# uingei/hevc

Hardware: AMD Instinct MI355X
Metric: encoded 1080p30 frames/sec/GPU; PSNR-Y parity vs libx265 at matched bitrate (higher is better)
Workload: dtype u8; 1 GPU; 1920x1080@30 SDR 8-bit Main, crf 19 capped by VBV maxrate 2940 kbps / bufsize 3528 kbit (the reference's libx265 operating point), 300-frame synthetic 'motion' clip per GPU, keyint 90 (4 closed GOPs of equal length), IPPP, full-search +-15, one clip per GPU, input resident in HBM

## Files before the change

hevc_amd/csrc/kernels/inter.h:

```cpp
#pragma once
#include "common.h"
#include "residual.h"

namespace mihevc {

template <typename T> struct InterArgs {
    Plane<const T> src[3];
    Plane<const T> ref[3];
    Plane<T> rec[3];
    int w, h, ctus_w;
    CostParams prm;
    const int16_t *centers;
    int32_t *me;
    mihevc_cu_rec *cu;
    int16_t *coef[3];
    unsigned long long *est;
    int sparse_coef;
    IpInfo *ip;
    Plane<const T> ref1[3];
    const int16_t *centers1;
    int32_t *me1;
};
template <typename T> DEV InterArgs<T> list1_view(const InterArgs<T> &a)
{
    InterArgs<T> b = a;
    for (int i = 0; i < 3; i++) b.ref[i] = a.ref1[i];
    b.centers = a.centers1; b.me = a.me1;
    return b;
}

DEVCONST int8_t kOff[9][2] = {{0, 0}, {-1, -1}, {0, -1}, {1, -1}, {-1, 0}, {1, 0}, {-1, 1}, {0, 1}, {1, 1}};
DEVCONST int8_t kRingSlot[8] = {4, 5, 2, 7, 1, 3, 6, 8};

template <typename T> struct PreArgs {
    Plane<const T> src, ref;
    uint8_t *lsrc, *lref;
    int w, h, bit_depth;
    int16_t *centers;
    unsigned *cost;
};
template <typename T> DEV void lowres_sample(const PreArgs<T> &a, int i)
{
    const int lw = a.w >> 2, n = lw * (a.h >> 2), sh = a.bit_depth - 8;
    if (i >= 2 * n) return;
    const Plane<const T> &p = i < n ? a.src : a.ref;
    const int k = i < n ? i : i - n, x = k % lw, y = k / lw;
    int s = 8 << sh;
#pragma unroll
    for (int j = 0; j < 4; j++) {
        const T *row = p.p + (ptrdiff_t)(4 * y + j) * p.stride + 4 * x;
        if (sizeof(T) == 1) {
            s = (int)sad_packed_u8(load_u32(row), 0u, (uint32_t)s);
        } else
            s += (int)row[0] + (int)row[1] + (int)row[2] + (int)row[3];
    }
    s >>= 4 + sh;
    (i < n ? a.lsrc : a.lref)[k] = (uint8_t)(s < 255 ? s : 255);
}
constexpr int PRE_SPAN = 2 * PRE_RANGE + 1;
constexpr int PRE_WIN_W = 40;
constexpr int PRE_WIN_STRIDE = 96;
struct PreShared {
    uint8_t blk[64];
    uint8_t win[(8 + 2 * PRE_RANGE) * PRE_WIN_STRIDE + 16];
    unsigned long long best;
    unsigned sad0;
};
template <typename T, class Ex> DEV void pre_search_program(Ex &ex, PreShared &s, const PreArgs<T> &a, int ctu)
{
    constexpr int R = PRE_RANGE, span = PRE_SPAN;
    const int lw = a.w >> 2, lh = a.h >> 2, wc = (lw + 7) >> 3, cx = ctu % wc, cy = ctu / wc;
    const int bw = lw - 8 * cx < 8 ? lw - 8 * cx : 8, bh = lh - 8 * cy < 8 ? lh - 8 * cy : 8;
    ex.phase([&](int tid) {
        if (tid < 64) { const int x = tid & 7, y = tid >> 3; s.blk[tid] = (x < bw && y < bh) ? a.lsrc[(8 * cy + y) * lw + 8 * cx + x] : (uint8_t)0; }
        if (8 * cx - R >= 0 && 8 * cx - R + PRE_WIN_W <= lw && 8 * cy - R >= 0 && 8 * cy + 8 + R <= lh) {
            constexpr int DPR = PRE_WIN_W / 4, ND = (8 + 2 * PRE_RANGE) * DPR, IT = (ND + NT - 1) / NT;
            uint32_t v[IT];
#pragma unroll
            for (int k = 0; k < IT; k++) {
                const int i = tid + k * NT;
                if (i < ND) v[k] = load_u32(a.lref + (size_t)(8 * cy - R + i / DPR) * lw + 8 * cx - R + 4 * (i % DPR));
            }
#pragma unroll
            for (int k = 0; k < IT; k++) {
                const int i = tid + k * NT;
                if (i < ND) store_u32_aligned(s.win + (i / DPR) * PRE_WIN_STRIDE + 4 * (i % DPR), v[k]);
            }
        } else {
            constexpr int NW = (8 + 2 * PRE_RANGE) * PRE_WIN_W, IT = (NW + NT - 1) / NT;
            uint8_t v[IT];
#pragma unroll
            for (int k = 0; k < IT; k++) {
                const int i = tid + k * NT;
                if (i < NW) v[k] = a.lref[clip3(0, lh - 1, 8 * cy + i / PRE_WIN_W - R) * lw + clip3(0, lw - 1, 8 * cx + i % PRE_WIN_W - R)];
            }
#pragma unroll
            for (int k = 0; k < IT; k++) {
                const int i = tid + k * NT;
                if (i < NW) s.win[(i / PRE_WIN_W) * PRE_WIN_STRIDE + i % PRE_WIN_W] = v[k];
            }
        }
        if (tid == 0) s.best = ~0ull;
    });
    ex.phase([&](int tid) {
        unsigned long long best = ~0ull;
        if (bw == 8 && bh == 8) {
            if (tid < 8 * span) {
                const int q = tid & 7, dyi = tid >> 3;
                uint64_t acc = 0;
#pragma unroll
                for (int y = 0; y < 8; y++) {
                    const uint8_t *w = s.win + (y + dyi) * PRE_WIN_STRIDE + 4 * q;
                    const uint32_t r0 = load_u32_aligned(w), r1 = load_u32_aligned(w + 4), r2 = load_u32_aligned(w + 8);
                    acc = qsad_u8(((uint64_t)r1 << 32) | r0, load_u32_aligned(s.blk + 8 * y), acc);
                    acc = qsad_u8(((uint64_t)r2 << 32) | r1, load_u32_aligned(s.blk + 8 * y + 4), acc);
                }
#pragma unroll
                for (int j = 0; j < 4; j++) {
                    const int dxi = 4 * q + j;
                    if (dxi >= span) continue;
                    const unsigned sad = (unsigned)((acc >> (16 * j)) & 0xffff);
                    if (dxi == R && dyi == R) s.sad0 = sad;
                    const unsigned long long key = ((unsigned long long)(4 * sad + (unsigned)(iabs(dxi - R) + iabs(dyi - R))) << 12) | (unsigned)(dyi * span + dxi);
                    best = key < best ? key : best;
                }
            }
        } else {
            for (int p = tid; p < span * span; p += NT) {
                const int dxi = p % span, dyi = p / span;
                unsigned sad = 0;
                for (int y = 0; y < bh; y++)
                    for (int x = 0; x < bw; x++) sad += (unsigned)iabs((int)s.blk[y * 8 + x] - (int)s.win[(y + dyi) * PRE_WIN_STRIDE + x + dxi]);
                if (dxi == R && dyi == R) s.sad0 = sad;
                const unsigned long long key = ((unsigned long long)(4 * sad + (unsigned)(iabs(dxi - R) + iabs(dyi - R))) << 12) | (unsigned)p;
                best = key < best ? key : best;
            }
        }
        if (best != ~0ull) ex.atomic_min(&s.best, best);
    });
    ex.phase([&](int tid) {
        if (tid != 0) return;
        int p = (int)(s.best & 4095);
        const unsigned sad_best = (unsigned)(((s.best >> 12) - (unsigned)(iabs(p % span - R) + iabs(p / span - R))) >> 2);
        if (2 * sad_best >= s.sad0) p = R * span + R;
        a.centers[2 * ctu] = (int16_t)(4 * (p % span - R));
        a.centers[2 * ctu + 1] = (int16_t)(4 * (p / span - R));
        if (a.cost) a.cost[ctu] = sad_best;
    });
}

DEV bool mv_rows_ok(int y, int n, int my, int h, int top, int bottom)
{
    const int ly0 = y + (my >> 2) - ((my & 3) ? 3 : 0), ly1 = y + n - 1 + (my >> 2) + ((my & 3) ? 4 : 0);
    const int cy0 = (y >> 1) + (my >> 3) - ((my & 7) ? 1 : 0), cy1 = (y >> 1) + (n >> 1) - 1 + (my >> 3) + ((my & 7) ? 2 : 0);
    if (top && (ly0 < 0 || cy0 < 0)) return false;
    if (bottom && (ly1 > h - 1 || cy1 > (h >> 1) - 1)) return false;
    return true;
}
DEV int clamp_center_y(int sy, int y0, int R, int h, int top, int bottom)
{
    const int ctu_h = h - y0 < CTU ? h - y0 : CTU;
    if (bottom && sy > h - (y0 + ctu_h) - R) sy = h - (y0 + ctu_h) - R;
    if (top && sy < R - y0) sy = R - y0;
    return sy;
}

template <typename T> struct MeShared {
    uint8_t src[32 * 32];
    unsigned long long best[21];
    uint8_t valid[21];
    unsigned nodeok[2 * MAX_RANGE + 1];
};
HDI int me_spanx(int R) { return ((2 * R + 1) + 3) & ~3; }
HDI int me_win_w(int R) { return 32 + me_spanx(R); }
HDI int me_win_stride(int R)
{
    int u = (me_win_w(R) + 4 + 3) >> 2;
    while ((u & 15) != 8) u++;
    return u << 2;
}
HDI int me_win_elems(int R) { return (32 + 2 * R) * me_win_stride(R) + 16; }

DEV void quad_block_row(const uint8_t *src, const uint8_t *ref, int ws, unsigned (&out)[4][4])
{
    uint64_t acc[4] = {0, 0, 0, 0};
// ... 143 lines not shown
                o[0] = 4 * (sx + p % spanx - R); o[1] = 4 * (sy + p / spanx - R); o[2] = (int32_t)(s.best[tid] >> 16);
            } else { o[0] = 0; o[1] = 0; o[2] = -1; }
        }
    });
}

template <typename T> struct InterShared {
    ResidualShared rs;
    T src[1536];
    T pred[1536];
    int mvx[21], mvy[21];
    unsigned cost[21];
    uint8_t valid[21];
    int satd[3][1][16];
    unsigned nsum[21];
    unsigned fsum[8][21];
    unsigned long long rbest[21];
    unsigned j16[4];
    int use16[4], use32;
    uint8_t alias[3][16];
    int tile_mvx[16], tile_mvy[16];
    uint8_t tile_node[16];
    uint8_t chosen[21];
    unsigned est;
    unsigned ip_cost, ip_act, ip_tiles;
    unsigned long long ip_sse;
    unsigned tu_dc[3][16], tu_dz[3][16], tu_bits[3][16], tu_zero[3];
};
constexpr int FRAC_PAIR_SUM = 8 * NT;
constexpr int FRAC_SCRATCH = FRAC_PAIR_SUM + NT;
static_assert(FRAC_SCRATCH <= (int)(sizeof(ResidualShared::scratch) / 4), "the fractional search's exchange must fit rs.scratch");
HDI int mc_win_y(int R) { return (32 + 2 * (R + 3) + 8 + 3) & ~3; }
HDI int mc_win_y_stride(int R) { return mc_win_y(R) + 4; }
HDI int mc_win_c(int R) { return (16 + (R + 3) + 8 + 3) & ~3; }
HDI int mc_win_c_stride(int R) { return mc_win_c(R) + 4; }
template <typename T> HDI size_t mc_win_y_bytes(int R) { return ((size_t)mc_win_y(R) * mc_win_y_stride(R) + 16) * sizeof(T); }
template <typename T> HDI size_t mc_win_c_bytes(int R) { return ((size_t)mc_win_c(R) * mc_win_c_stride(R) + 16) * sizeof(T); }
HDI constexpr size_t align16(size_t v) { return (v + 15) & ~(size_t)15; }

struct BiShared {
    int mx0[21], my0[21];
    unsigned c0[21], cb[21];
    uint8_t mode[21];
    uint8_t tile_mode[16];
    int tile_mv1x[16], tile_mv1y[16];
    alignas(16) int16_t p0[1536];
};

struct InterLds { size_t y, u, v, bytes; };
template <typename T> HDI constexpr size_t inter_win_in() { return offsetof(InterShared<T>, rs) + offsetof(ResidualShared, scratch) + 4 * (size_t)FRAC_SCRATCH; }
template <typename T> HDI constexpr size_t inter_win_out() { return align16(sizeof(InterShared<T>)); }
template <typename T> HDI InterLds inter_lds(int R)
{
    const size_t n[3] = {mc_win_y_bytes<T>(R), mc_win_c_bytes<T>(R), mc_win_c_bytes<T>(R)};
    const size_t hi = offsetof(InterShared<T>, rs) + offsetof(ResidualShared, scratch) + sizeof(ResidualShared::scratch);
    size_t in = inter_win_in<T>(), out = inter_win_out<T>(), at[3];
    for (int i = 0; i < 3; i++) {
        const size_t r = align16(n[i]);
        if (in + r <= hi) { at[i] = in; in += r; } else { at[i] = out; out += r; }
    }
    return InterLds{at[0], at[1], at[2], out};
}
struct InterBLds { size_t y, u, v, bi, bytes; };
template <typename T> HDI InterBLds inter_b_lds(int R)
{
    InterBLds l;
    l.y = inter_win_out<T>();
    l.u = l.y + align16(mc_win_y_bytes<T>(R));
    l.v = l.u + align16(mc_win_c_bytes<T>(R));
    l.bi = l.v + align16(mc_win_c_bytes<T>(R));
    l.bytes = l.bi + align16(sizeof(BiShared));
    return l;
}

struct TapBytes { uint32_t lo, hi; };
struct TapPairs { uint32_t p[4]; };
DEV TapBytes tap_bytes(int f) { return TapBytes{load_u32(&g_tab.luma_tap[f][0]), load_u32(&g_tab.luma_tap[f][4])}; }
DEV TapPairs tap_pairs(int f)
{
    TapPairs t;
#pragma unroll
    for (int k = 0; k < 4; k++) t.p[k] = pack_lo16(g_tab.luma_tap[f][2 * k], g_tab.luma_tap[f][2 * k + 1]);
    return t;
}
template <typename T> DEV auto row_taps(int f)
{
    if constexpr (sizeof(T) == 1) return tap_bytes(f); else return tap_pairs(f);
}

DEV void luma_row4(const uint8_t *win, int idx, const TapBytes &t, int, int (&hv)[4])
{
    const int off = idx & 3;
    const uint8_t *p = win + (idx - off);
    uint32_t d[4], q[3];
#pragma unroll
    for (int k = 0; k < 4; k++) d[k] = load_u32_aligned(p + 4 * k);
#pragma unroll
    for (int k = 0; k < 3; k++) q[k] = align_bytes(d[k + 1], d[k], off) ^ 0x80808080u;
    hv[0] = dot4_i8(q[0], t.lo, dot4_i8(q[1], t.hi, 128 * 64));
#pragma unroll
    for (int i = 1; i < 4; i++) hv[i] = dot4_i8(align_bytes(q[1], q[0], i), t.lo, dot4_i8(align_bytes(q[2], q[1], i), t.hi, 128 * 64));
}
DEV void luma_row4(const uint16_t *win, int idx, const TapPairs &t, int shift1, int (&hv)[4])
{
    const int off = idx & 1;
    const uint16_t *p = win + (idx - off);
    uint32_t d[7], e[6], o[5];
#pragma unroll
    for (int k = 0; k < 7; k++) d[k] = load_u32_aligned(p + 2 * k);
#pragma unroll
    for (int k = 0; k < 6; k++) e[k] = align_bytes(d[k + 1], d[k], 2 * off);
#pragma unroll
    for (int k = 0; k < 5; k++) o[k] = align_bytes(e[k + 1], e[k], 2);
#pragma unroll
    for (int i = 0; i < 4; i++) {
        int v = 0;
#pragma unroll
        for (int k = 0; k < 4; k++) v = dot2_i16((i & 1) ? o[(i >> 1) + k] : e[(i >> 1) + k], t.p[k], v);
        hv[i] = v >> shift1;
    }
}

template <typename T> DEV void luma_quad14(const T *win, int i00, int ws, int fx, int fy, int bit_depth, int (&out)[4])
{
    const auto tx = row_taps<T>(fx);
    const int8_t *ty = g_tab.luma_tap[fy];
    int acc[4] = {0, 0, 0, 0};
#pragma unroll
    for (int r = 0; r < 8; r++) {
        int hv[4];
        luma_row4(win, i00 + (r - 3) * ws - 3, tx, bit_depth - 8, hv);
        const int t = ty[r];
#pragma unroll
        for (int i = 0; i < 4; i++) acc[i] += t * hv[i];
    }
#pragma unroll
    for (int i = 0; i < 4; i++) out[i] = acc[i] >> 6;
}
template <typename T> DEV int chroma_sample14(const T *p00, int ws, int fx, int fy, int bit_depth)
{
    const int8_t *tx = g_tab.chroma_tap[fx], *ty = g_tab.chroma_tap[fy];
    const int shift1 = bit_depth - 8;
    int acc = 0;
    for (int r = 0; r < 4; r++) {
        const T *row = p00 + (r - 1) * ws - 1;
        int v = tx[0] * row[0] + tx[1] * row[1] + tx[2] * row[2] + tx[3] * row[3];
        acc += ty[r] * (v >> shift1);
    }
    return acc >> 6;
}
DEV int weighted_uni(int p, int bit_depth) { const int sh = 14 - bit_depth; return clip3(0, (1 << bit_depth) - 1, (p + (1 << (sh - 1))) >> sh); }
DEV int weighted_bi(int p0, int p1, int bit_depth) { const int sh = 15 - bit_depth; return clip3(0, (1 << bit_depth) - 1, (p0 + p1 + (1 << (sh - 1))) >> sh); }

DEV void luma_col_pair(int r, const int (&hv)[4], int (&prev)[4], const TapPairs &ty, int (&acc)[8][4])
{
    if (r > 0) {
#pragma unroll
        for (int i = 0; i < 4; i++) {
            const uint32_t pr = pack_lo16(prev[i], hv[i]);
#pragma unroll
            for (int k = 0; k < 4; k++) {
                const int j = r - 1 - 2 * k;
                if (j >= 0 && j < 8) acc[j][i] = dot2_i16(pr, ty.p[k], acc[j][i]);
            }
        }
    }
#pragma unroll
    for (int i = 0; i < 4; i++) prev[i] = hv[i];
}
DEV void luma_half_diff(const uint8_t *win, int i00, int ws, int fx, int fy, int, const uint8_t *src, int src_stride, int (&m)[8][4])
{
    const TapBytes tx = tap_bytes(fx);
    if (wave_all(fy == 0)) {
#pragma unroll
        for (int j = 0; j < 8; j++) {
            int hv[4];
            luma_row4(win, i00 + j * ws - 3, tx, 0, hv);
            const uint32_t w = load_u32_aligned(src + j * src_stride);
#pragma unroll
            for (int i = 0; i < 4; i++) m[j][i] = (int)((w >> (8 * i)) & 255) - clip3(0, 255, (hv[i] + 32) >> 6);
        }
        return;
    }
    if (wave_all(fx == 0)) {
        const TapBytes ty = tap_bytes(fy);
        const int idx = i00 - 3 * ws, off = idx & 3;
        uint32_t rows[15];
#pragma unroll
        for (int r = 0; r < 15; r++) {
            const uint8_t *p = win + (idx - off) + r * ws;
            rows[r] = align_bytes(load_u32_aligned(p + 4), load_u32_aligned(p), off) ^ 0x80808080u;
        }
        uint32_t col[4][4];
#pragma unroll
        for (int g = 0; g < 4; g++) {
            const uint32_t r4[4] = {rows[4 * g], rows[4 * g + 1], rows[4 * g + 2], g < 3 ? rows[4 * g + 3] : 0u};
            transpose_bytes4(r4, col[g]);
        }
#pragma unroll
        for (int j = 0; j < 8; j++) {
            const int g = j >> 2, sh = j & 3;
            const uint32_t w = load_u32_aligned(src + j * src_stride);
#pragma unroll
            for (int i = 0; i < 4; i++) {
                const uint32_t lo = align_bytes(col[g + 1][i], col[g][i], sh), hi = align_bytes(col[g + 2][i], col[g + 1][i], sh);
                const int v = dot4_i8(lo, ty.lo, dot4_i8(hi, ty.hi, 128 * 64));
                m[j][i] = (int)((w >> (8 * i)) & 255) - clip3(0, 255, (v + 32) >> 6);
            }
        }
        return;
    }
    const TapPairs ty = tap_pairs(fy);
    int acc[8][4], prev[4];
#pragma unroll
    for (int j = 0; j < 8; j++)
#pragma unroll
        for (int i = 0; i < 4; i++) acc[j][i] = 0;
#pragma unroll
    for (int r = 0; r < 15; r++) {
        int hv[4];
        luma_row4(win, i00 + (r - 3) * ws - 3, tx, 0, hv);
        luma_col_pair(r, hv, prev, ty, acc);
    }
#pragma unroll
    for (int j = 0; j < 8; j++) {
        const uint32_t w = load_u32_aligned(src + j * src_stride);
#pragma unroll
        for (int i = 0; i < 4; i++) m[j][i] = (int)((w >> (8 * i)) & 255) - clip3(0, 255, ((acc[j][i] >> 6) + 32) >> 6);
    }
}
DEV void luma_half_diff(const uint16_t *win, int i00, int ws, int fx, int fy, int bit_depth, const uint16_t *src, int src_stride, int (&m)[8][4])
{
    const TapPairs tx = tap_pairs(fx), ty = tap_pairs(fy);
    const int shift1 = bit_depth - 8, shift3 = 14 - bit_depth, maxv = (1 << bit_depth) - 1, off3 = 1 << (shift3 - 1);
    if (wave_all(fy == 0)) {
#pragma unroll
        for (int j = 0; j < 8; j++) {
            int hv[4];
            luma_row4(win, i00 + j * ws - 3, tx, shift1, hv);
#pragma unroll
            for (int i = 0; i < 4; i++) m[j][i] = (int)src[j * src_stride + i] - clip3(0, maxv, (hv[i] + off3) >> shift3);
        }
        return;
    }
    const bool v_only = wave_all(fx == 0);
    int acc[8][4], prev[4];
#pragma unroll
    for (int j = 0; j < 8; j++)
#pragma unroll
        for (int i = 0; i < 4; i++) acc[j][i] = 0;
#pragma unroll
    for (int r = 0; r < 15; r++) {
        int hv[4];
        if (v_only) {
#pragma unroll
            for (int i = 0; i < 4; i++) hv[i] = (int)win[i00 + (r - 3) * ws + i] << (6 - shift1);
        } else luma_row4(win, i00 + (r - 3) * ws - 3, tx, shift1, hv);
        luma_col_pair(r, hv, prev, ty, acc);
    }
#pragma unroll
    for (int j = 0; j < 8; j++)
#pragma unroll
        for (int i = 0; i < 4; i++) m[j][i] = (int)src[j * src_stride + i] - clip3(0, maxv, ((acc[j][i] >> 6) + off3) >> shift3);
}
DEV void hadamard_half(int (&m)[8][4])
{
#pragma unroll
    for (int x = 0; x < 4; x++)
#pragma unroll
        for (int st = 1; st < 8; st <<= 1)
#pragma unroll
            for (int i = 0; i < 8; i++)
                if (!(i & st)) { int p = m[i][x], q = m[i + st][x]; m[i][x] = p + q; m[i + st][x] = p - q; }
#pragma unroll
    for (int y = 0; y < 8; y++) {
        const int p0 = m[y][0] + m[y][1], p1 = m[y][0] - m[y][1], p2 = m[y][2] + m[y][3], p3 = m[y][2] - m[y][3];
        m[y][0] = p0 + p2; m[y][1] = p1 + p3; m[y][2] = p0 - p2; m[y][3] = p1 - p3;
    }
}

template <typename T> DEV int luma_tile_int(const T *win, int i00, int ws, const T *src, int src_stride)
{
    int m[8][8];
#pragma unroll
    for (int j = 0; j < 8; j++) {
        int px[8];
        load_row8(win, i00 + j * ws, px);
#pragma unroll
        for (int i = 0; i < 8; i++) m[j][i] = (int)src[j * src_stride + i] - px[i];
    }
    return hadamard8_satd(m);
}

template <typename T, class Ex, bool BI = false>
DEV void inter_ctu_program(Ex &ex, InterShared<T> &s, T *win_y, T *win_u, T *win_v, const InterArgs<T> &a, int ctu, BiShared *bsh = nullptr)
{
    const int R0 = a.prm.me_range, R = R0 + 3, bd = a.prm.bit_depth, lam = a.prm.lambda_sad_q4;
    const int x0 = (ctu % a.ctus_w) * CTU, y0 = (ctu / a.ctus_w) * CTU;
    const int mct = a.prm.mc_top, mcb = a.prm.mc_bottom;
    const int sx = wave_uniform(a.centers ? a.centers[2 * ctu] : 0), sy0 = wave_uniform(a.centers ? a.centers[2 * ctu + 1] : 0);
    const int sy = (mct || mcb) ? clamp_center_y(sy0, y0, R0, a.h, mct, mcb) : sy0;
    const int wy = mc_win_y(R0), wys = mc_win_y_stride(R0), wc = mc_win_c(R0), wcs = mc_win_c_stride(R0);
    const int oy_x = x0 + sx - R - 4, oy_y = y0 + sy - R - 4;
    const int oc_x = (x0 >> 1) + ((4 * sx - 4 * R - 3) >> 3) - 1, oc_y = (y0 >> 1) + ((4 * sy - 4 * R - 3) >> 3) - 1;

    ex.phase([&](int tid) {
        residual_init_lane(s.rs, tid);
        load_ctu_source<T>(s.src, a.src, x0, y0, a.w, a.h, tid);
        copy_window<T>(win_y, wys, a.ref[0].p, a.ref[0].stride, oy_x, oy_y, wy, wy, -PAD_Y, a.w + PAD_Y - 1, -PAD_Y, a.h + PAD_Y - 1, tid);
        copy_window<T>(win_u, wcs, a.ref[1].p, a.ref[1].stride, oc_x, oc_y, wc, wc, -PAD_C, (a.w >> 1) + PAD_C - 1, -PAD_C, (a.h >> 1) + PAD_C - 1, tid);
        copy_window<T>(win_v, wcs, a.ref[2].p, a.ref[2].stride, oc_x, oc_y, wc, wc, -PAD_C, (a.w >> 1) + PAD_C - 1, -PAD_C, (a.h >> 1) + PAD_C - 1, tid);
        if (tid < 21) {
            const int32_t *m = a.me + ((size_t)ctu * 21 + tid) * 3;
            s.mvx[tid] = m[0]; s.mvy[tid] = m[1]; s.valid[tid] = m[2] >= 0; s.cost[tid] = 0; s.nsum[tid] = 0;
        }
    });
    ex.phase([&](int tid) {
        for (int u = tid; u < 3 * 16; u += NT) {
            int level = u >> 4, t = u & 15;
            int txp = t & 3, typ = t >> 2, node = node_of_tile(level, txp, typ);
            if (!s.valid[node]) continue;
            int al = level;
            for (int fl = 2; fl > level; fl--) {
                int fn = node_of_tile(fl, txp, typ);
                if (s.valid[fn] && s.mvx[fn] == s.mvx[node] && s.mvy[fn] == s.mvy[node]) { al = fl; break; }
            }
            s.alias[level][t] = (uint8_t)al;
            if (al != level) continue;
            int px = x0 + txp * 8 + (s.mvx[node] >> 2) - oy_x, py = y0 + typ * 8 + (s.mvy[node] >> 2) - oy_y;
            s.satd[level][0][t] = luma_tile_int<T>(win_y, py * wys + px, wys, s.src + typ * 8 * 32 + txp * 8, 32);
        }
    });
    ex.phase([&](int tid) {
        if (tid < 3 * 16) {
            const int level = tid >> 4, t = tid & 15, node = node_of_tile(level, t & 3, t >> 2);
            if (s.valid[node]) ex.atomic_add(&s.nsum[node], (unsigned)s.satd[s.alias[level][t]][0][t]);
        }
        if (tid >= 64 && tid < 64 + 8 * 21) s.fsum[(tid - 64) / 21][(tid - 64) % 21] = 0;
    });
    ex.wave_step([&](int tid) {
        if (tid >= 21) return;
        s.chosen[tid] = 0;
        s.cost[tid] = s.valid[tid] ? (s.nsum[tid] << 4) + (unsigned)(lam * (mvd_bits(s.mvx[tid] - 4 * sx) + mvd_bits(s.mvy[tid] - 4 * sy))) : 0;
        if (tid == 0) { s.est = 0; s.ip_cost = 0; s.ip_act = 0; s.ip_tiles = 0; s.ip_sse = 0; }
    });
    ex.wave_step([&](int tid) {
        if (tid >= 4) return;
        const int q = tid;
        unsigned js = (unsigned)(lam * 2);
        for (int t = 0; t < 4; t++) if (s.valid[5 + 4 * q + t]) js += s.cost[5 + 4 * q + t] + (unsigned)(lam * 4);
        const unsigned jw = s.cost[1 + q] + (unsigned)(lam * 4);
        s.use16[q] = s.valid[1 + q] && jw <= js;
        s.j16[q] = s.use16[q] ? jw : js;
    });
    ex.wave_step([&](int tid) {
        if (tid != 0) return;
        const unsigned js32 = (unsigned)(lam * 2) + s.j16[0] + s.j16[1] + s.j16[2] + s.j16[3];
        s.use32 = s.valid[0] && s.cost[0] + (unsigned)(lam * 4) <= js32;
    });
    ex.phase([&](int tid) {
        if (tid >= 16) return;
        const int t = tid, txp = t & 3, typ = t >> 2, q = (typ >> 1) * 2 + (txp >> 1), n8 = node_of_tile(2, txp, typ);
        const int node = s.use32 ? 0 : s.use16[q] ? 1 + q : n8, inside = s.valid[n8];
        s.tile_node[t] = (uint8_t)node;
        if (inside) s.chosen[node] = 1;
        s.rs.tu_log2[t] = inside ? (uint8_t)(node == 0 ? 5 : node < 5 ? 4 : 3) : 0;
        s.rs.tu_intra[t] = 0;
    });
    auto refine = [&](const int csx, const int csy, const int wox, const int woy) {
    for (int round = 0; round < 2; round++) {
        const int step = round == 0 ? 2 : 1;
        struct Kept { uint32_t v[2][4]; };
        wave_chain(ex, [&](int tid) -> Kept {
            const int u = tid >> 1, half = tid & 1, k = kRingSlot[u >> 4], t = u & 15;
            Kept kept{};
            if (!s.rs.tu_log2[t]) return kept;
            const int txp = t & 3, typ = t >> 2, node = s.tile_node[t];
            const int mx = s.mvx[node] + kOff[k][0] * step, my = s.mvy[node] + kOff[k][1] * step;
            const int px = x0 + txp * 8 + 4 * half + (mx >> 2) - wox, py = y0 + typ * 8 + (my >> 2) - woy;
            int m[8][4];
            luma_half_diff((const T *)win_y, py * wys + px, wys, mx & 3, my & 3, bd, (const T *)(s.src + typ * 8 * 32 + txp * 8 + 4 * half), 32, m);
            {
                uint32_t P[4][4];
#pragma unroll
                for (int r2 = 0; r2 < 4; r2++)
#pragma unroll
                    for (int c = 0; c < 4; c++) P[r2][c] = perm_bytes((uint32_t)m[2 * r2 + 1][c], (uint32_t)m[2 * r2][c], 0x05040100u);
#pragma unroll
                for (int c = 0; c < 4; c++) {
                    const uint32_t a0 = pk_add16(P[0][c], P[1][c]), a1 = pk_sub16(P[0][c], P[1][c]), a2 = pk_add16(P[2][c], P[3][c]), a3 = pk_sub16(P[2][c], P[3][c]);
                    P[0][c] = pk_add16(a0, a2); P[1][c] = pk_add16(a1, a3); P[2][c] = pk_sub16(a0, a2); P[3][c] = pk_sub16(a1, a3);
                }
                uint32_t o[4][4];
#pragma unroll
                for (int r2 = 0; r2 < 4; r2++) {
                    const uint32_t p0 = pk_add16(P[r2][0], P[r2][1]), p1 = pk_sub16(P[r2][0], P[r2][1]), p2 = pk_add16(P[r2][2], P[r2][3]), p3 = pk_sub16(P[r2][2], P[r2][3]);
                    o[r2][0] = pk_add16(p0, p2); o[r2][1] = pk_add16(p1, p3); o[r2][2] = pk_sub16(p0, p2); o[r2][3] = pk_sub16(p1, p3);
                }
                uint32_t *x = s.rs.scratch + tid * 8;
                const int sw = ((tid >> 2) ^ (tid >> 3)) & 1;
#pragma unroll
                for (int c = 0; c < 2; c++) {
                    uint32_t send[4];
#pragma unroll
                    for (int i = 0; i < 4; i++) { kept.v[c][i] = half ? o[2 + c][i] : o[c][i]; send[i] = half ? o[c][i] : o[2 + c][i]; }
                    store_x4(x + 4 * (c ^ sw), send);
                }
            }
            return kept;
        }, [&](int tid, const Kept &kept) {
            const int u = tid >> 1, t = u & 15;
            if (!s.rs.tu_log2[t]) return;
            const uint32_t *xp = s.rs.scratch + (tid ^ 1) * 8;
            const int sw = ((tid >> 2) ^ (tid >> 3)) & 1;
            unsigned sum = 0;
            {
                uint32_t acc[2] = {0, 0};
#pragma unroll
                for (int c = 0; c < 2; c++) {
                    uint32_t vb[4];
                    load_x4(xp + 4 * (c ^ sw), vb);
                    const uint32_t (&va)[4] = kept.v[c];
#pragma unroll
                    for (int i = 0; i < 4; i++) {
#pragma unroll
                        for (int sgn = 0; sgn < 2; sgn++) {
                            const uint32_t v = sgn ? pk_sub16(va[i], vb[i]) : pk_add16(va[i], vb[i]);
                            const uint32_t av = pk_max_i16(v, pk_sub16(0u, v));
                            const uint32_t mx = pk_max_i16(av, (av >> 16) | (av << 16));
                            if constexpr (sizeof(T) == 1) acc[c] = pk_add16(acc[c], mx); else sum += mx & 0xffffu;
                        }
                    }
                }
                if constexpr (sizeof(T) == 1) sum = (acc[0] & 0xffffu) + (acc[1] & 0xffffu);
                s.rs.scratch[FRAC_PAIR_SUM + tid] = 2u * sum;
            }
        });
        ex.phase([&](int tid) {
            const int u = tid >> 1, k = kRingSlot[u >> 4], t = u & 15;
            if (tid >= 1 && tid < 43 && (tid & 1)) s.rbest[tid >> 1] = (unsigned long long)s.cost[tid >> 1] << 4;
            if ((tid & 1) || !s.rs.tu_log2[t]) return;
            const unsigned satd = (s.rs.scratch[FRAC_PAIR_SUM + tid] + s.rs.scratch[FRAC_PAIR_SUM + tid + 1] + 2) >> 2;
            ex.atomic_add(&s.fsum[k - 1][s.tile_node[t]], satd);
        });
        ex.phase([&](int tid) {
            const int node = tid >> 3, k = 1 + (tid & 7);
            if (node >= 21 || !s.valid[node] || !s.chosen[node]) return;
            const unsigned satd = s.fsum[k - 1][node];
            s.fsum[k - 1][node] = 0;
            const int mx = s.mvx[node] + kOff[k][0] * step, my = s.mvy[node] + kOff[k][1] * step;
            if (mct || mcb) {
                int nx, ny, nl;
                node_geom(node, nx, ny, nl);
                if (!mv_rows_ok(y0 + ny, 1 << nl, my, a.h, mct, mcb)) return;
            }
            const unsigned c = (satd << 4) + (unsigned)(lam * (mvd_bits(mx - 4 * csx) + mvd_bits(my - 4 * csy)));
            ex.atomic_min(&s.rbest[node], ((unsigned long long)c << 4) | (unsigned)k);
        });
        ex.phase([&](int tid) {
            if (tid >= 21 || !s.valid[tid] || !s.chosen[tid]) return;
            const unsigned long long best = s.rbest[tid];
            const int k = (int)(best & 15);
            s.mvx[tid] += kOff[k][0] * step; s.mvy[tid] += kOff[k][1] * step;
            s.cost[tid] = (unsigned)(best >> 4);
        });
    }
    };
    refine(sx, sy, oy_x, oy_y);
    auto lane_at = [](int tid) { return ((tid >> 6) * 8 + ((tid >> 1) & 7)) * 32 + ((tid >> 4) & 3) * 8 + (tid & 1) * 4; };
    auto luma14 = [&](int tid, int wox, int woy, int (&v)[4]) {
        const int t = tid >> 4, node = s.tile_node[t], mx = s.mvx[node], my = s.mvy[node];
        const int px = x0 + (t & 3) * 8 + (tid & 1) * 4 + (mx >> 2) - wox, py = y0 + (t >> 2) * 8 + ((tid >> 1) & 7) + (my >> 2) - woy;
        luma_quad14<T>(win_y, py * wys + px, wys, mx & 3, my & 3, bd, v);
    };
    auto chroma_tile = [](int i) { return ((i >> 6) & 3) * 4 + ((i >> 2) & 3); };
    auto chroma14 = [&](int i, int cox, int coy) {
        const int x = i & 15, y = (i >> 4) & 15, node = s.tile_node[chroma_tile(i)], mx = s.mvx[node], my = s.mvy[node];
        const int px = (x0 >> 1) + x + (mx >> 3) - cox, py = (y0 >> 1) + y + (my >> 3) - coy;
        return chroma_sample14<T>((i >> 8 ? win_v : win_u) + py * wcs + px, wcs, mx & 7, my & 7, bd);
    };
    if constexpr (BI) {
        BiShared &b = *bsh;
        const int sx1 = a.centers1 ? a.centers1[2 * ctu] : 0, sy1 = a.centers1 ? a.centers1[2 * ctu + 1] : 0;
        const int o1_x = x0 + sx1 - R - 4, o1_y = y0 + sy1 - R - 4;
        const int oc1_x = (x0 >> 1) + ((4 * sx1 - 4 * R - 3) >> 3) - 1, oc1_y = (y0 >> 1) + ((4 * sy1 - 4 * R - 3) >> 3) - 1;
        ex.phase([&](int tid) {
            if (tid < 21) { b.mx0[tid] = s.mvx[tid]; b.my0[tid] = s.mvy[tid]; b.c0[tid] = s.cost[tid]; b.cb[tid] = 0; }
            if (s.rs.tu_log2[tid >> 4]) {
                int v[4];
                luma14(tid, oy_x, oy_y, v);
#pragma unroll
                for (int i = 0; i < 4; i++) b.p0[lane_at(tid) + i] = (int16_t)v[i];
            }
            for (int i = tid; i < 512; i += NT)
                if (s.rs.tu_log2[chroma_tile(i)]) b.p0[1024 + i] = (int16_t)chroma14(i, oc_x, oc_y);
        });
        ex.phase([&](int tid) {
            copy_window<T>(win_y, wys, a.ref1[0].p, a.ref1[0].stride, o1_x, o1_y, wy, wy, -PAD_Y, a.w + PAD_Y - 1, -PAD_Y, a.h + PAD_Y - 1, tid);
            copy_window<T>(win_u, wcs, a.ref1[1].p, a.ref1[1].stride, oc1_x, oc1_y, wc, wc, -PAD_C, (a.w >> 1) + PAD_C - 1, -PAD_C, (a.h >> 1) + PAD_C - 1, tid);
            copy_window<T>(win_v, wcs, a.ref1[2].p, a.ref1[2].stride, oc1_x, oc1_y, wc, wc, -PAD_C, (a.w >> 1) + PAD_C - 1, -PAD_C, (a.h >> 1) + PAD_C - 1, tid);
            if (tid < 21) {
                const int32_t *m = a.me1 + ((size_t)ctu * 21 + tid) * 3;
                s.mvx[tid] = m[0]; s.mvy[tid] = m[1]; s.nsum[tid] = 0;
            }
        });
        ex.phase([&](int tid) {
            if (tid >= 16 || !s.rs.tu_log2[tid]) return;
            const int t = tid, txp = t & 3, typ = t >> 2, node = s.tile_node[t];
            const int px = x0 + txp * 8 + (s.mvx[node] >> 2) - o1_x, py = y0 + typ * 8 + (s.mvy[node] >> 2) - o1_y;
            ex.atomic_add(&s.nsum[node], (unsigned)luma_tile_int<T>(win_y, py * wys + px, wys, s.src + typ * 8 * 32 + txp * 8, 32));
        });
        ex.phase([&](int tid) {
            if (tid < 21 && s.valid[tid] && s.chosen[tid])
                s.cost[tid] = (s.nsum[tid] << 4) + (unsigned)(lam * (mvd_bits(s.mvx[tid] - 4 * sx1) + mvd_bits(s.mvy[tid] - 4 * sy1)));
        });
        refine(sx1, sy1, o1_x, o1_y);
        ex.phase([&](int tid) {
            if (!s.rs.tu_log2[tid >> 4]) return;
            int v[4];
            luma14(tid, o1_x, o1_y, v);
#pragma unroll
            for (int i = 0; i < 4; i++) {
                const int at = lane_at(tid) + i;
                s.rs.scratch[4 * tid + i] = (uint32_t)((int)s.src[at] - weighted_bi((int)b.p0[at], v[i], bd));
            }
        });
        ex.phase([&](int tid) {
            if (tid >= 16 || !s.rs.tu_log2[tid]) return;
            int m[8][8];
#pragma unroll
            for (int j = 0; j < 8; j++)
#pragma unroll
                for (int i = 0; i < 8; i++) m[j][i] = (int)s.rs.scratch[tid * 64 + j * 8 + i];
            ex.atomic_add(&b.cb[s.tile_node[tid]], (unsigned)hadamard8_satd(m));
        });
        ex.phase([&](int tid) {
            if (tid >= 21 || !s.valid[tid] || !s.chosen[tid]) return;
            const unsigned bits0 = (unsigned)(mvd_bits(b.mx0[tid] - 4 * sx) + mvd_bits(b.my0[tid] - 4 * sy)), bits1 = (unsigned)(mvd_bits(s.mvx[tid] - 4 * sx1) + mvd_bits(s.mvy[tid] - 4 * sy1));
            const unsigned cbi = (b.cb[tid] << 4) + (unsigned)lam * (bits0 + bits1);
            const unsigned long long k0 = (((unsigned long long)b.c0[tid] + (unsigned long long)(lam * 2)) << 2) | 0, k1 = (((unsigned long long)s.cost[tid] + (unsigned long long)(lam * 2)) << 2) | 1,
                                     k2 = (((unsigned long long)cbi + (unsigned long long)lam) << 2) | 2;
            const unsigned long long kb = k0 <= k1 ? (k0 <= k2 ? k0 : k2) : (k1 <= k2 ? k1 : k2);
            b.mode[tid] = (uint8_t)(kb & 3);
        });
        ex.phase([&](int tid) {
            if (tid < 16) {
                const int node = s.tile_node[tid], mode = b.mode[node];
                b.tile_mode[tid] = (uint8_t)mode;
                s.tile_mvx[tid] = mode != 1 ? b.mx0[node] : 0; s.tile_mvy[tid] = mode != 1 ? b.my0[node] : 0;
                b.tile_mv1x[tid] = mode != 0 ? s.mvx[node] : 0; b.tile_mv1y[tid] = mode != 0 ? s.mvy[node] : 0;
            }
            if (s.rs.tu_log2[tid >> 4]) {
                const int mode = b.mode[s.tile_node[tid >> 4]];
                int v[4] = {0, 0, 0, 0};
                if (mode != 0) luma14(tid, o1_x, o1_y, v);
#pragma unroll
                for (int i = 0; i < 4; i++) {
                    const int at = lane_at(tid) + i, p0 = (int)b.p0[at];
                    s.pred[at] = (T)(mode == 0 ? weighted_uni(p0, bd) : mode == 1 ? weighted_uni(v[i], bd) : weighted_bi(p0, v[i], bd));
                }
            }
            for (int i = tid; i < 512; i += NT) {
                if (!s.rs.tu_log2[chroma_tile(i)]) continue;
                const int mode = b.mode[s.tile_node[chroma_tile(i)]], p0 = (int)b.p0[1024 + i], p1 = mode != 0 ? chroma14(i, oc1_x, oc1_y) : 0;
                s.pred[1024 + i] = (T)(mode == 0 ? weighted_uni(p0, bd) : mode == 1 ? weighted_uni(p1, bd) : weighted_bi(p0, p1, bd));
            }
        });
    }
    if (!BI && a.ip)
    ex.phase([&](int tid) {
        if (tid >= 64 && tid < 85 && s.valid[tid - 64] && s.chosen[tid - 64]) ex.atomic_add(&s.ip_cost, s.cost[tid - 64]);
        if (tid >= 128 && tid < 144 && s.rs.tu_log2[tid - 128]) ex.atomic_add(&s.ip_tiles, 1u);
    });
    if (!BI && a.ip && s.ip_cost >= ((4u * 64u * s.ip_tiles) << 4)) {
        ex.phase([&](int tid) {
            if (tid >= 16 || !s.rs.tu_log2[tid]) return;
            const T *sp = s.src + (tid >> 2) * 8 * 32 + (tid & 3) * 8;
            int m[8][8];
#pragma unroll
            for (int j = 0; j < 8; j++)
#pragma unroll
                for (int i = 0; i < 8; i++) m[j][i] = (int)sp[j * 32 + i];
            ex.atomic_add(&s.ip_act, (unsigned)hadamard8_ac(m));
        });
    }
    if constexpr (!BI)
    ex.phase([&](int tid) {
        if (tid < 16) { s.tile_mvx[tid] = s.mvx[s.tile_node[tid]]; s.tile_mvy[tid] = s.mvy[s.tile_node[tid]]; }
        if (s.rs.tu_log2[tid >> 4]) {
            int v[4];
            luma14(tid, oy_x, oy_y, v);
#pragma unroll
            for (int i = 0; i < 4; i++) s.pred[lane_at(tid) + i] = (T)weighted_uni(v[i], bd);
        }
        for (int i = tid; i < 512; i += NT)
            if (s.rs.tu_log2[chroma_tile(i)]) s.pred[1024 + i] = (T)weighted_uni(chroma14(i, oc_x, oc_y), bd);
// ... 118 lines not shown
```

Before: 5974 frames/s.

## Pair vertically adjacent refine candidates to share one 9-row interpolated prediction

For 8-bit input in the first (step-2) fractional refine round, candidates whose MVs differ by one integer row (step 2 in quarter-pel = half... paired via kPairJob) share a single 9-row interpolated prediction, producing two SATDs from one filter pass. A dedicated vertical-only path uses byte transposes and dot4 for fx==0. Work is redistributed so fewer lanes do double jobs, with a per-CTU rotation of lane assignment to balance load across waves. This adds register pressure and extra scratch slots, and the interpolation rounding path for pairs differs slightly from the original.

Result: no change. 5938 frames/s (-0.6%).

```diff
diff --git a/hevc_amd/csrc/kernels/inter.h b/hevc_amd/csrc/kernels/inter.h
--- a/hevc_amd/csrc/kernels/inter.h
+++ b/hevc_amd/csrc/kernels/inter.h
@@ -31,6 +31,7 @@
 
 DEVCONST int8_t kOff[9][2] = {{0, 0}, {-1, -1}, {0, -1}, {1, -1}, {-1, 0}, {1, 0}, {-1, 1}, {0, 1}, {1, 1}};
 DEVCONST int8_t kRingSlot[8] = {4, 5, 2, 7, 1, 3, 6, 8};
+DEVCONST int8_t kPairJob[8][2] = {{1, 6}, {3, 8}, {2, 7}, {0, 0}, {4, 0}, {5, 0}, {0, 0}, {0, 0}};
 
 template <typename T> struct PreArgs {
     Plane<const T> src, ref;
@@ -480,7 +481,7 @@
 DEV int weighted_uni(int p, int bit_depth) { const int sh = 14 - bit_depth; return clip3(0, (1 << bit_depth) - 1, (p + (1 << (sh - 1))) >> sh); }
 DEV int weighted_bi(int p0, int p1, int bit_depth) { const int sh = 15 - bit_depth; return clip3(0, (1 << bit_depth) - 1, (p0 + p1 + (1 << (sh - 1))) >> sh); }
 
-DEV void luma_col_pair(int r, const int (&hv)[4], int (&prev)[4], const TapPairs &ty, int (&acc)[8][4])
+template <int N> DEV void luma_col_pair(int r, const int (&hv)[4], int (&prev)[4], const TapPairs &ty, int (&acc)[N][4])
 {
     if (r > 0) {
 #pragma unroll
@@ -489,7 +490,7 @@
 #pragma unroll
             for (int k = 0; k < 4; k++) {
                 const int j = r - 1 - 2 * k;
-                if (j >= 0 && j < 8) acc[j][i] = dot2_i16(pr, ty.p[k], acc[j][i]);
+                if (j >= 0 && j < N) acc[j][i] = dot2_i16(pr, ty.p[k], acc[j][i]);
             }
         }
     }
@@ -590,6 +591,66 @@
     for (int j = 0; j < 8; j++)
 #pragma unroll
         for (int i = 0; i < 4; i++) m[j][i] = (int)src[j * src_stride + i] - clip3(0, maxv, ((acc[j][i] >> 6) + off3) >> shift3);
+}
+DEV void luma_pair_pred(const uint8_t *win, int i00, int ws, int fx, int fy, uint32_t (&pr)[9])
+{
+    if (wave_all(fx == 0)) {
+        const TapBytes ty = tap_bytes(fy);
+        const int idx = i00 - 3 * ws, off = idx & 3;
+        uint32_t col[4][4];
+#pragma unroll
+        for (int g = 0; g < 4; g++) {
+            uint32_t r4[4];
+#pragma unroll
+            for (int r = 0; r < 4; r++) {
+                const uint8_t *p = win + (idx - off) + (4 * g + r) * ws;
+                r4[r] = align_bytes(load_u32_aligned(p + 4), load_u32_aligned(p), off) ^ 0x80808080u;
+            }
+            transpose_bytes4(r4, col[g]);
+        }
+#pragma unroll
+        for (int j = 0; j < 9; j++) {
+            const int g = j >> 2, sh = j & 3;
+            uint32_t out = 0;
+#pragma unroll
+            for (int i = 0; i < 4; i++) {
+                const uint32_t lo = align_bytes(col[g + 1][i], col[g][i], sh), hi = g < 2 ? align_bytes(col[g + 2][i], col[g + 1][i], sh) : col[g + 1][i];
+                const int v = dot4_i8(lo, ty.lo, dot4_i8(hi, ty.hi, 128 * 64));
+                out |= (uint32_t)clip3(0, 255, (v + 32) >> 6) << (8 * i);
+            }
+            pr[j] = out;
+        }
+        return;
+    }
+    const TapBytes tx = tap_bytes(fx);
+    const TapPairs ty = tap_pairs(fy);
+    int acc[9][4], prev[4];
+#pragma unroll
+    for (int j = 0; j < 9; j++)
+#pragma unroll
+        for (int i = 0; i < 4; i++) acc[j][i] = 0;
+#pragma unroll
+    for (int r = 0; r < 16; r++) {
+        int hv[4];
+        luma_row4(win, i00 + (r - 3) * ws - 3, tx, 0, hv);
+        luma_col_pair(r, hv, prev, ty, acc);
+    }
+#pragma unroll
+    for (int j = 0; j < 9; j++) {
+        uint32_t out = 0;
+#pragma unroll
+        for (int i = 0; i < 4; i++) out |= (uint32_t)clip3(0, 255, ((acc[j][i] >> 6) + 32) >> 6) << (8 * i);
+        pr[j] = out;
+    }
+}
+DEV void pair_diff(const uint32_t (&pr)[9], int lower, const uint8_t *src, int src_stride, int (&m)[8][4])
+{
+#pragma unroll
+    for (int j = 0; j < 8; j++) {
+        const uint32_t w = load_u32_aligned(src + j * src_stride), p = lower ? pr[j + 1] : pr[j];
+#pragma unroll
+        for (int i = 0; i < 4; i++) m[j][i] = (int)((w >> (8 * i)) & 255) - (int)((p >> (8 * i)) & 255);
+    }
 }
 DEV void hadamard_half(int (&m)[8][4])
 {
@@ -696,80 +757,113 @@
         s.rs.tu_intra[t] = 0;
     });
     auto refine = [&](const int csx, const int csy, const int wox, const int woy) {
+    auto had_send = [&](int slot, int half, const int (&m)[8][4], uint32_t (&keep)[2][4]) {
+        uint32_t P[4][4];
+#pragma unroll
+        for (int r2 = 0; r2 < 4; r2++)
+#pragma unroll
+            for (int c = 0; c < 4; c++) P[r2][c] = perm_bytes((uint32_t)m[2 * r2 + 1][c], (uint32_t)m[2 * r2][c], 0x05040100u);
+#pragma unroll
+        for (int c = 0; c < 4; c++) {
+            const uint32_t a0 = pk_add16(P[0][c], P[1][c]), a1 = pk_sub16(P[0][c], P[1][c]), a2 = pk_add16(P[2][c], P[3][c]), a3 = pk_sub16(P[2][c], P[3][c]);
+            P[0][c] = pk_add16(a0, a2); P[1][c] = pk_add16(a1, a3); P[2][c] = pk_sub16(a0, a2); P[3][c] = pk_sub16(a1, a3);
+        }
+        uint32_t o[4][4];
+#pragma unroll
+        for (int r2 = 0; r2 < 4; r2++) {
+            const uint32_t p0 = pk_add16(P[r2][0], P[r2][1]), p1 = pk_sub16(P[r2][0], P[r2][1]), p2 = pk_add16(P[r2][2], P[r2][3]), p3 = pk_sub16(P[r2][2], P[r2][3]);
+            o[r2][0] = pk_add16(p0, p2); o[r2][1] = pk_add16(p1, p3); o[r2][2] = pk_sub16(p0, p2); o[r2][3] = pk_sub16(p1, p3);
+        }
+        uint32_t *x = s.rs.scratch + slot * 8;
+        const int sw = ((slot >> 2) ^ (slot >> 3)) & 1;
+#pragma unroll
+        for (int c = 0; c < 2; c++) {
+            uint32_t send[4];
+#pragma unroll
+            for (int i = 0; i < 4; i++) { keep[c][i] = half ? o[2 + c][i] : o[c][i]; send[i] = half ? o[c][i] : o[2 + c][i]; }
+            store_x4(x + 4 * (c ^ sw), send);
+        }
+    };
+    auto had_recv = [&](int slot, const uint32_t (&keep)[2][4]) {
+        const uint32_t *xp = s.rs.scratch + (slot ^ 1) * 8;
+        const int sw = ((slot >> 2) ^ (slot >> 3)) & 1;
+        unsigned sum = 0;
+        uint32_t acc[2] = {0, 0};
+#pragma unroll
+        for (int c = 0; c < 2; c++) {
+            uint32_t vb[4];
+            load_x4(xp + 4 * (c ^ sw), vb);
+            const uint32_t (&va)[4] = keep[c];
+#pragma unroll
+            for (int i = 0; i < 4; i++) {
+#pragma unroll
+                for (int sgn = 0; sgn < 2; sgn++) {
+                    const uint32_t v = sgn ? pk_sub16(va[i], vb[i]) : pk_add16(va[i], vb[i]);
+                    const uint32_t av = pk_max_i16(v, pk_sub16(0u, v));
+                    const uint32_t mx = pk_max_i16(av, (av >> 16) | (av << 16));
+                    if constexpr (sizeof(T) == 1) acc[c] = pk_add16(acc[c], mx); else sum += mx & 0xffffu;
+                }
+            }
+        }
+        if constexpr (sizeof(T) == 1) sum = (acc[0] & 0xffffu) + (acc[1] & 0xffffu);
+        s.rs.scratch[FRAC_PAIR_SUM + slot] = 2u * sum;
+    };
     for (int round = 0; round < 2; round++) {
         const int step = round == 0 ? 2 : 1;
-        struct Kept { uint32_t v[2][4]; };
+        constexpr bool kPairs = sizeof(T) == 1;
+        struct Job { int t, k0, k1; };
+        auto job_of = [&](int tid) {
+            const int t = (tid >> 1) & 15;
+            if (kPairs && round == 0) return Job{t, kPairJob[tid >> 5][0], kPairJob[tid >> 5][1]};
+            return Job{t, kRingSlot[tid >> 5], 0};
+        };
+        auto slot1 = [](int tid) { return tid + (tid < 64 ? 192 : 32); };
+        const int turn = (kPairs && round == 0) ? 64 * (int)(((unsigned)ctu * 0x9E3779B1u) >> 30) : 0;
+        auto job_lane = [&](int tid) { return (tid + turn) & (NT - 1); };
+        struct Kept { uint32_t v[kPairs ? 2 : 1][2][4]; };
         wave_chain(ex, [&](int tid) -> Kept {
-            const int u = tid >> 1, half = tid & 1, k = kRingSlot[u >> 4], t = u & 15;
+            tid = job_lane(tid);
+            const Job j = job_of(tid);
+            const int half = tid & 1, t = j.t;
             Kept kept{};
-            if (!s.rs.tu_log2[t]) return kept;
+            if (!j.k0 || !s.rs.tu_log2[t]) return kept;
             const int txp = t & 3, typ = t >> 2, node = s.tile_node[t];
-            const int mx = s.mvx[node] + kOff[k][0] * step, my = s.mvy[node] + kOff[k][1] * step;
+            const int mx = s.mvx[node] + kOff[j.k0][0] * step, my = s.mvy[node] + kOff[j.k0][1] * step;
             const int px = x0 + txp * 8 + 4 * half + (mx >> 2) - wox, py = y0 + typ * 8 + (my >> 2) - woy;
+            const T *src = (const T *)(s.src + typ * 8 * 32 + txp * 8 + 4 * half);
             int m[8][4];
-            luma_half_diff((const T *)win_y, py * wys + px, wys, mx & 3, my & 3, bd, (const T *)(s.src + typ * 8 * 32 + txp * 8 + 4 * half), 32, m);
-            {
-                uint32_t P[4][4];
-#pragma unroll
-                for (int r2 = 0; r2 < 4; r2++)
-#pragma unroll
-                    for (int c = 0; c < 4; c++) P[r2][c] = perm_bytes((uint32_t)m[2 * r2 + 1][c], (uint32_t)m[2 * r2][c], 0x05040100u);
-#pragma unroll
-                for (int c = 0; c < 4; c++) {
-                    const uint32_t a0 = pk_add16(P[0][c], P[1][c]), a1 = pk_sub16(P[0][c], P[1][c]), a2 = pk_add16(P[2][c], P[3][c]), a3 = pk_sub16(P[2][c], P[3][c]);
-                    P[0][c] = pk_add16(a0, a2); P[1][c] = pk_add16(a1, a3); P[2][c] = pk_sub16(a0, a2); P[3][c] = pk_sub16(a1, a3);
+            if constexpr (kPairs) {
+                if (j.k1) {
+                    uint32_t pr[9];
+                    luma_pair_pred((const T *)win_y, py * wys + px, wys, mx & 3, my & 3, pr);
+                    pair_diff(pr, 0, src, 32, m);
+                    had_send(tid, half, m, kept.v[0]);
+                    pair_diff(pr, 1, src, 32, m);
+                    had_send(slot1(tid), half, m, kept.v[1]);
+                    return kept;
                 }
-                uint32_t o[4][4];
-#pragma unroll
-                for (int r2 = 0; r2 < 4; r2++) {
-                    const uint32_t p0 = pk_add16(P[r2][0], P[r2][1]), p1 = pk_sub16(P[r2][0], P[r2][1]), p2 = pk_add16(P[r2][2], P[r2][3]), p3 = pk_sub16(P[r2][2], P[r2][3]);
-                    o[r2][0] = pk_add16(p0, p2); o[r2][1] = pk_add16(p1, p3); o[r2][2] = pk_sub16(p0, p2); o[r2][3] = pk_sub16(p1, p3);
-                }
-                uint32_t *x = s.rs.scratch + tid * 8;
-                const int sw = ((tid >> 2) ^ (tid >> 3)) & 1;
-#pragma unroll
-                for (int c = 0; c < 2; c++) {
-                    uint32_t send[4];
-#pragma unroll
-                    for (int i = 0; i < 4; i++) { kept.v[c][i] = half ? o[2 + c][i] : o[c][i]; send[i] = half ? o[c][i] : o[2 + c][i]; }
-                    store_x4(x + 4 * (c ^ sw), send);
-                }
-            }
+            }
+            luma_half_diff((const T *)win_y, py * wys + px, wys, mx & 3, my & 3, bd, src, 32, m);
+            had_send(tid, half, m, kept.v[0]);
             return kept;
         }, [&](int tid, const Kept &kept) {
-            const int u = tid >> 1, t = u & 15;
-            if (!s.rs.tu_log2[t]) return;
-            const uint32_t *xp = s.rs.scratch + (tid ^ 1) * 8;
-            const int sw = ((tid >> 2) ^ (tid >> 3)) & 1;
-            unsigned sum = 0;
-            {
-                uint32_t acc[2] = {0, 0};
-#pragma unroll
-                for (int c = 0; c < 2; c++) {
-                    uint32_t vb[4];
-                    load_x4(xp + 4 * (c ^ sw), vb);
-                    const uint32_t (&va)[4] = kept.v[c];
-#pragma unroll
-                    for (int i = 0; i < 4; i++) {
-#pragma unroll
-                        for (int sgn = 0; sgn < 2; sgn++) {
-                            const uint32_t v = sgn ? pk_sub16(va[i], vb[i]) : pk_add16(va[i], vb[i]);
-                            const uint32_t av = pk_max_i16(v, pk_sub16(0u, v));
-                            const uint32_t mx = pk_max_i16(av, (av >> 16) | (av << 16));
-                            if constexpr (sizeof(T) == 1) acc[c] = pk_add16(acc[c], mx); else sum += mx & 0xffffu;
-                        }
-                    }
-                }
-                if constexpr (sizeof(T) == 1) sum = (acc[0] & 0xffffu) + (acc[1] & 0xffffu);
-                s.rs.scratch[FRAC_PAIR_SUM + tid] = 2u * sum;
-            }
-        });
-        ex.phase([&](int tid) {
-            const int u = tid >> 1, k = kRingSlot[u >> 4], t = u & 15;
+            tid = job_lane(tid);
+            const Job j = job_of(tid);
+            if (!j.k0 || !s.rs.tu_log2[j.t]) return;
+            had_recv(tid, kept.v[0]);
+            if constexpr (kPairs) if (j.k1) had_recv(slot1(tid), kept.v[1]);
+        });
+        ex.phase([&](int tid) {
             if (tid >= 1 && tid < 43 && (tid & 1)) s.rbest[tid >> 1] = (unsigned long long)s.cost[tid >> 1] << 4;
-            if ((tid & 1) || !s.rs.tu_log2[t]) return;
-            const unsigned satd = (s.rs.scratch[FRAC_PAIR_SUM + tid] + s.rs.scratch[FRAC_PAIR_SUM + tid + 1] + 2) >> 2;
-            ex.atomic_add(&s.fsum[k - 1][s.tile_node[t]], satd);
+            tid = job_lane(tid);
+            const Job j = job_of(tid);
+            if ((tid & 1) || !j.k0 || !s.rs.tu_log2[j.t]) return;
+            auto add = [&](int k, int slot) {
+                const unsigned satd = (s.rs.scratch[FRAC_PAIR_SUM + slot] + s.rs.scratch[FRAC_PAIR_SUM + slot + 1] + 2) >> 2;
+                ex.atomic_add(&s.fsum[k - 1][s.tile_node[j.t]], satd);
+            };
+            add(j.k0, tid);
+            if (j.k1) add(j.k1, slot1(tid));
         });
         ex.phase([&](int tid) {
             const int node = tid >> 3, k = 1 + (tid & 7);
```
